# joaospinto/sip_optimal_control

Hardware: AMD Instinct MI355X
Metric: Riccati sweeps/sec (backward+forward) (higher is better)
Workload: dtype f64

## Files before the change

sip_optimal_control_amd/csrc/chain_qw16.hpp:

```cpp
#pragma once
#include <hip/hip_runtime.h>
#include <type_traits>

#include "dpp_blocks_gen.hpp"

namespace sipamd {

template <int I, int E, class F>
__device__ __forceinline__ void sfor(F &&f) {
  if constexpr (I < E) {
    f(std::integral_constant<int, I>{});
    sfor<I + 1, E>(f);
  }
}
template <int I, int E, class F>
__device__ __forceinline__ void sfor_down(F &&f) {
  if constexpr (I > E) {
    f(std::integral_constant<int, I>{});
    sfor_down<I - 1, E>(f);
  }
}

template <int K>
__device__ __forceinline__ double bcast(double x) {
  double und;
  asm volatile("" : "=v"(und));
  return __builtin_amdgcn_update_dpp(und, x, 0x150 + K, 0xf, 0xf, false);
}

__device__ __forceinline__ double rsqrt_nr(double d) {
  const double y = __builtin_amdgcn_rsq(d);
  const double s = d * y;
  const double e = __builtin_fma(-s, y, 1.0);
  const double t = __builtin_fma(0.375, e, 0.5);
  return __builtin_fma(y * e, t, y);
}

__device__ __forceinline__ double rcp_nr(double d) {
  const double y = __builtin_amdgcn_rcp(d);
  const double e = __builtin_fma(-d, y, 1.0);
  const double t = __builtin_fma(e, e, e);
  return __builtin_fma(y, t, y);
}

template <int S>
__device__ __forceinline__ bool chol_ldl_dpp(double (&A)[S], double (&dinv)[S],
                                             const int c) {
#ifdef SIP_QW16_CHOL_SELECT
  unsigned long long failmask = 0;
  sfor<0, S>([&](auto kk) {
    constexpr int k = decltype(kk)::value;
    const double d = bcast<k>(A[k]);
    failmask |= __ballot(d <= 0.0);
    const double y2 = rcp_nr(d);
    dinv[k] = y2;
    const double upd = (c > k && c < S) ? A[k] * y2 : 0.0;
    rank1<S - k - 1, k, true, false>(A + k + 1, A + k + 1, upd);
  });
  return ((failmask >> (__lane_id() & 63)) & 1ull) != 0;
#else
  double dmin = __builtin_inf();
  sfor<0, S>([&](auto kk) {
    constexpr int k = decltype(kk)::value;
    const double d = bcast<k>(A[k]);
    asm("v_min_f64 %0, %1, %2" : "=v"(dmin) : "v"(dmin), "v"(d));
    const double own = A[k] * ((c > k && c < S) ? 1.0 : 0.0);
    const double y2 = rcp_nr(d);
    dinv[k] = y2;
    const double upd = own * y2;
    rank1<S - k - 1, k, true, false>(A + k + 1, A + k + 1, upd);
  });
  return dmin <= 0.0;
#endif
}

template <int S>
__device__ __forceinline__ void ldl_solve_dpp(const double (&Lt)[S],
                                              const double (&dinv)[S],
                                              double (&X)[S]) {
  sfor<0, S>([&](auto jj) {
    constexpr int j = decltype(jj)::value;
    X[j] *= dinv[j];
    rank1<S - j - 1, j, true, (j == 0)>(X + j + 1, Lt + j + 1, X[j]);
  });
  double acc[S];
  sfor<0, S>([&](auto jj) { acc[decltype(jj)::value] = 0.0; });
  sfor_down<S - 1, -1>([&](auto jj) {
    constexpr int j = decltype(jj)::value;
    X[j] = __builtin_fma(-dinv[j], acc[j], X[j]);
    spread<j, false, false>(acc, Lt[j], X[j]);
  });
}

template <int N, int M, bool SYM = false>
struct ChainLayout {
  static constexpr int QLEN = SYM ? N * (N + 1) / 2 : N * N;
  static constexpr int RLEN = SYM ? M * (M + 1) / 2 : M * M;
  static constexpr int NODE = QLEN + N;
  static constexpr int EDGE = N * N + 2 * N * M + RLEN;
  static constexpr int VNODE = 2 * N;
  static constexpr int VEDGE = M;
  static constexpr int GAIN = M * N + M;
  static constexpr int WSN = N * N + 2 * N;
};

template <int N, bool EXPORT = false>
__device__ __forceinline__ bool node_factor(const double (&V)[N], const double dl,
                                            const int c, const double (&E)[N],
                                            const double (&tv)[N], double (&W)[N],
                                            double (&X)[N], double *Lt = nullptr) {
  const double sdi = rsqrt_nr(dl);
  const double sd = dl * sdi;
  double S[N], A[N], rinv[N];
  sfor<0, N>([&](auto ii) { S[decltype(ii)::value] = 0.0; });
  spread<N, false, true>(S, sd, sd);
  sfor<0, N>([&](auto ii) {
    constexpr int r = decltype(ii)::value;
    A[r] = __builtin_fma(S[r], V[r], E[r]);
  });
  const bool fail = chol_ldl_dpp<N>(A, rinv, c);
  if constexpr (EXPORT)
    sfor<0, N>([&](auto ii) { Lt[decltype(ii)::value] = A[decltype(ii)::value]; });
  sfor<0, N>([&](auto ii) { X[decltype(ii)::value] = E[decltype(ii)::value]; });
  spreadv<N, false>(X, sdi, tv);
  ldl_solve_dpp<N>(A, rinv, X);
  sfor<0, N>([&](auto ii) { S[decltype(ii)::value] = 0.0; });
  spread<N, false, true>(S, sdi, sdi);
  sfor<0, N>([&](auto ii) {
    constexpr int r = decltype(ii)::value;
    W[r] = (E[r] - X[r]) * S[r];
  });
  return fail;
}

#ifndef SIP_LQR_NT_SOL
#define SIP_LQR_NT_SOL 0
#endif
#ifndef SIP_LQR_NT_IN
#define SIP_LQR_NT_IN 2
#endif
#ifndef SIP_LQR_NT_FAB
#define SIP_LQR_NT_FAB SIP_LQR_NT_IN
#endif
#ifndef SIP_LQR_NT_FSP
#define SIP_LQR_NT_FSP 0
#endif
typedef __attribute__((address_space(3))) char lds_char;
typedef const __attribute__((address_space(3))) double lds_cdouble;

#ifdef SIP_LQR_STAMPS
#define SIP_STAMP(var)                                                         \
  do {                                                                         \
    __builtin_amdgcn_sched_barrier(0);                                         \
    asm volatile("s_memtime %0\n\ts_waitcnt lgkmcnt(0)" : "=s"(var)::"memory"); \
    __builtin_amdgcn_sched_barrier(0);                                         \
  } while (0)
#define SIP_STAMP_ARG , unsigned long long *__restrict__ stamps
#define SIP_SEG(k)                                                             \
  do {                                                                         \
    unsigned long long now_;                                                   \
    SIP_STAMP(now_);                                                           \
    seg[k] += now_ - seg_last;                                                 \
    seg_last = now_;                                                           \
  } while (0)
#else
#define SIP_SEG(k)                                                             \
  do {                                                                         \
  } while (0)
#define SIP_STAMP(var)                                                         \
  do {                                                                         \
  } while (0)
#define SIP_STAMP_ARG
#endif

template <int PIECES>
struct StageDma {
  static constexpr int INSTR = (4 * PIECES + 63) / 64;
  static constexpr int BYTES = INSTR * 1024;
  static constexpr int ROW_BYTES = PIECES * 16;
#ifdef SIP_QW16_DMA_PLAIN
  static constexpr int GROUP = 1;
#else
  static constexpr int GROUP = 4;
#endif
  static constexpr unsigned BIAS = (GROUP - 1) * 1024u;
  unsigned off[INSTR > 0 ? INSTR : 1];
  __device__ __forceinline__ void init(const int lane,
                                       const unsigned problem_stride_bytes,
                                       const unsigned max_rel) {
    sfor<0, INSTR>([&](auto jj) {
      constexpr int j = decltype(jj)::value;
      const unsigned q = (unsigned)(j * 64 + lane) < 4u * PIECES ? (unsigned)(j * 64 + lane) : 4u * PIECES - 1u;
      unsigned rr = q / PIECES;
      const unsigned within = q - rr * PIECES;
      rr = rr < max_rel ? rr : max_rel;
      off[j] = rr * problem_stride_bytes + within * 16u + BIAS - (unsigned)(j % GROUP) * 1024u;
    });
  }
  template <int AUX = 0>
  __device__ __forceinline__ void issue(const char *base, lds_char *dst,
                                        const int lane) const {
    const char *lowered = base - BIAS;
    sfor<0, INSTR>([&](auto jj) {
      constexpr int j = decltype(jj)::value;
      __builtin_amdgcn_global_load_lds((const __attribute__((address_space(1))) void *)(lowered + off[j]),
                                       (__attribute__((address_space(3))) void *)(dst + (j - j % GROUP) * 1024), 16,
                                       (j % GROUP) * 1024, AUX);
    });
  }
};

template <int DWORDS>
struct StageDmaDwords {
  static constexpr int INSTR = (4 * DWORDS + 63) / 64;
  static constexpr int BYTES = (INSTR * 256 + 1023) / 1024 * 1024;
  static constexpr int ROW_BYTES = DWORDS * 4;
  unsigned off[INSTR > 0 ? INSTR : 1];
  __device__ __forceinline__ void init(const int lane, const unsigned problem_stride_bytes, const unsigned max_rel) {
    sfor<0, INSTR>([&](auto jj) {
      constexpr int j = decltype(jj)::value;
      const unsigned q = (unsigned)(j * 64 + lane) < 4u * DWORDS ? (unsigned)(j * 64 + lane) : 4u * DWORDS - 1u;
      unsigned rr = q / DWORDS;
      const unsigned within = q - rr * DWORDS;
      rr = rr < max_rel ? rr : max_rel;
      off[j] = rr * problem_stride_bytes + within * 4u;
    });
  }
  template <int AUX = 0>
  __device__ __forceinline__ void issue(const char *base, lds_char *dst, const int lane) const {
    sfor<0, INSTR>([&](auto jj) {
      constexpr int j = decltype(jj)::value;
      __builtin_amdgcn_global_load_lds((const __attribute__((address_space(1))) void *)(base + off[j]),
                                       (__attribute__((address_space(3))) void *)(dst + j * 256), 4, 0, AUX);
    });
  }
};

template <int PIECES>
struct StageDmaRows {
  static constexpr int IP = (PIECES + 63) / 64;
  static constexpr int INSTR = 4 * IP;
  static constexpr int ROW_BYTES = IP * 1024;
  static constexpr int BYTES = 4 * ROW_BYTES;
  static constexpr bool RAGGED = PIECES % 64 != 0;
  unsigned vo_main, vo_tail;
  unsigned long long row[4];
  __device__ __forceinline__ void init(const int lane,
                                       const unsigned problem_stride_bytes,
                                       const unsigned max_rel) {
    vo_main = (unsigned)lane * 16u;
    const unsigned last = (unsigned)(PIECES - 1 - 64 * (IP - 1));
    vo_tail = ((unsigned)lane < last ? (unsigned)lane : last) * 16u;
    sfor<0, 4>([&](auto rq) {
      constexpr unsigned r = decltype(rq)::value;
      row[r] = (unsigned long long)(r < max_rel ? r : max_rel) * problem_stride_bytes;
    });
  }
  template <int AUX = 0>
  __device__ __forceinline__ void issue(const char *base, lds_char *dst,
                                        const int lane) const {
    sfor<0, 4>([&](auto rq) {
      constexpr int r = decltype(rq)::value;
      const char *region = base + row[r];
      sfor<0, IP>([&](auto jq) {
        constexpr int jj = decltype(jq)::value;
        constexpr int g = jj / 4;
        const unsigned vo = (RAGGED && jj == IP - 1) ? vo_tail : vo_main;
        __builtin_amdgcn_global_load_lds(
            (const __attribute__((address_space(1))) void *)(region + g * 4096 + vo),
            (__attribute__((address_space(3))) void *)(dst + r * ROW_BYTES + g * 4096), 16, (jj % 4) * 1024, AUX);
      });
    });
  }
};

template <int N, int M, bool WPACK, bool SPLIT = false, bool SYM = false>
struct StagedCfg {
  using L = ChainLayout<N, M, SYM>;
  static_assert(!SYM || (L::QLEN % 2 == 0 && L::RLEN % 2 == 0 && N % 2 == 0 && M % 2 == 0),
                "the symmetric-packed kernels are instantiated where every block stays a whole number of 16-byte pieces");
  static constexpr int AB = N * N + N * M;
  static constexpr int STG = L::NODE + L::EDGE - (SPLIT ? AB : 0);
  static constexpr int WSN =
      WPACK ? ((N * (N + 1) / 2 + 2 * N + 1) / 2) * 2 : L::WSN;
  using BV = StageDma<(L::VNODE + L::VEDGE + 1) / 2>;
  using BMflat = StageDma<(STG + 1) / 2>;
  using BMrows = StageDmaRows<(STG + 1) / 2>;
  struct NoStream {
    static constexpr int INSTR = 0, BYTES = 0, ROW_BYTES = 0;
  };
  static_assert(!SPLIT || AB % 2 == 0, "the split kernels are instantiated for even N (A | B in whole 16-byte pieces)");
  using BA = std::conditional_t<SPLIT, StageDmaRows<AB / 2>, NoStream>;
  static constexpr int SCR_BYTES_ = ((4 * 2 * N + N) * 8 + 1023) / 1024 * 1024;
  static constexpr int waves_per_cu(int bm_bytes) {
    const int per_wave = 2 * (bm_bytes + BA::BYTES + BV::BYTES) + SCR_BYTES_;
    const int w = 163840 / per_wave;
    return w > 4 ? 4 : w;
  }
#ifdef SIP_QW16_DMA_FLAT
  using BM = BMflat;
#else
  using BM = std::conditional_t<SPLIT || waves_per_cu(BMrows::BYTES) >= waves_per_cu(BMflat::BYTES), BMrows, BMflat>;
#endif
  static constexpr int B_BYTES = BM::BYTES + BA::BYTES + BV::BYTES;
  using FA = StageDma<(N * N + N * M + 1) / 2>;
  using FG = std::conditional_t<L::GAIN % 2 == 0, StageDma<L::GAIN / 2>, StageDmaDwords<2 * L::GAIN>>;
  using FW = StageDma<WSN / 2>;
  using FC = std::conditional_t<N % 2 == 0, StageDma<N / 2>, StageDmaDwords<2 * N>>;
  static constexpr int F_BYTES = FA::BYTES + FG::BYTES + FW::BYTES + FC::BYTES;
  static constexpr int F_GLDS = FA::INSTR + FG::INSTR + FW::INSTR + FC::INSTR;
  static constexpr int B_NBUF = 2;
  static constexpr int lds_main(int fbufs) {
    return B_NBUF * B_BYTES > fbufs * F_BYTES ? B_NBUF * B_BYTES : fbufs * F_BYTES;
  }
  static constexpr int waves_with(int fbufs) {
    const int w = 163840 / (lds_main(fbufs) + SCR_BYTES_);
    return w > 4 ? 4 : w;
  }
#ifdef SIP_LQR_FNBUF
  static constexpr int F_NBUF = SIP_LQR_FNBUF;
#else
  static constexpr int F_NBUF = (waves_with(2) > waves_with(3) || lds_main(3) + SCR_BYTES_ > 65536) ? 2 : 3;
#endif
  static constexpr int LDS_MAIN = lds_main(F_NBUF);
  static constexpr int SCR_BYTES = ((4 * 2 * N + N) * 8 + 1023) / 1024 * 1024;
  static constexpr int LDS_BYTES = LDS_MAIN + SCR_BYTES;
  static constexpr bool OK = N <= 16;
  static constexpr bool WIDE = N % 2 == 0;
};

template <int N, int M, bool STAGED, bool WPACK, bool SPLIT = false, bool SYM = false>
__global__ __launch_bounds__(64) void chain_factor_solve_qw16(
    const double *__restrict__ mats, const double *__restrict__ vecs,
    double *__restrict__ sol, double *__restrict__ gains,
    double *__restrict__ wsp, int *__restrict__ status, const long batch,
    const int T, const int mode, double *__restrict__ gfac,
    const double *__restrict__ ab, const long ab_pstride, const long ab_sstride SIP_STAMP_ARG) {
  constexpr bool VDIST = N == 16;
  static_assert(N >= 1 && N <= 16, "one problem per 16-lane row");
  static_assert(M >= 1 && M <= 16, "");
  using L = ChainLayout<N, M, SYM>;
  using C = StagedCfg<N, M, WPACK, SPLIT, SYM>;
  static_assert(!SPLIT || (STAGED && WPACK), "the split kernel is the staged one");
  static_assert(!SYM || (STAGED && !VDIST), "the symmetric-packed layout is served by the staged kernels");
  unsigned long long ts_begin = 0, ts_term = 0, ts_bwd = 0, ts_root = 0,
                     ts_end = 0, ts_a = 0, ts_b = 0, acc_bwait = 0,
                     acc_fwait = 0;
  (void)ts_begin, (void)ts_term, (void)ts_bwd, (void)ts_root, (void)ts_end,
      (void)ts_a, (void)ts_b, (void)acc_bwait, (void)acc_fwait;
  unsigned long long seg[12] = {0, 0, 0, 0, 0, 0, 0, 0, 0, 0, 0, 0}, seg_last = 0;
  (void)seg, (void)seg_last;
  SIP_STAMP(ts_begin);
  static_assert(!STAGED || C::LDS_BYTES <= 65536, "the LDS images of this shape exceed a workgroup's 64 KiB");
  constexpr int STG = C::STG;
  constexpr int OFF_M = L::NODE + (SPLIT ? 0 : N * N + N * M), OFF_R = OFF_M + N * M;
  constexpr int VSTG = L::VNODE + L::VEDGE;
  constexpr int WSN = C::WSN;
  constexpr int WG = WPACK ? N * (N + 1) / 2 : N * N;

  extern __shared__ double lds_raw[];
  lds_char *const lds = (lds_char *)lds_raw;

  const int lane = threadIdx.x & 63;
  const int c = lane & 15;
  const int rr = lane >> 4;
  const long p0 = (long)blockIdx.x * 4;
  long p = p0 + rr;
  const bool valid = p < batch;
  if (!valid)
    p = batch - 1;
  const bool isM = c < N;
  const bool isV = c == N;
  const int cm = isM ? c : N - 1;
  const int cu = c < M ? c : M - 1;

  const long mats_len = (long)(T + 1) * L::NODE + (long)T * (STG - L::NODE);
  const long vecs_len = (long)(T + 1) * L::VNODE + (long)T * L::VEDGE;
  const long gains_len = (long)T * L::GAIN;
  const long ws_len = (long)(T + 1) * WSN;
  const double *pm = mats + p * mats_len;
  const double *pv = vecs + p * vecs_len;
  double *ps = sol + p * vecs_len;
  double *pg = gains + p * gains_len;
  double *pw = wsp + p * ws_len;
  const unsigned max_rel =
      (unsigned)((batch - 1 - p0) < 3 ? (batch - 1 - p0) : 3);

  double E[N];
  sfor<0, N>([&](auto ii) {
    constexpr int r = decltype(ii)::value;
    E[r] = (c == r) ? 1.0 : 0.0;
  });

  auto spill_row_offsets = [&](int(&woff)[N]) {
    sfor<0, N>([&](auto kk) {
      constexpr int k = decltype(kk)::value;
      if constexpr (WPACK) {
        const int lo = k < cm ? k : cm, hi = k < cm ? cm : k;
        woff[k] = lo * N - (lo * (lo - 1)) / 2 + (hi - lo);
      } else {
        woff[k] = cm * N + k;
      }
    });
  };

  int stat = 0;
  double W[N], V[N], t[N], vch[N];
  double vd = 0.0, td = 0.0, qd = 0.0;
  auto sum4 = [](const double (&a)[4]) { return (a[0] + a[1]) + (a[2] + a[3]); };

  const __amdgpu_buffer_rsrc_t ws_rsrc = __builtin_amdgcn_make_buffer_rsrc(
      (void *)(wsp + p0 * ws_len), 0, (int)((max_rel + 1) * ws_len * 8), 0x00020000);
  const int wstore_base = (valid && isM)
                              ? (int)(rr * ws_len * 8) + (c * N - (c * (c - 1)) / 2 - c) * 8
                              : 0x7ffff000;

  typedef __attribute__((address_space(3))) double lds_double;
  lds_char *const scr = lds + C::LDS_MAIN;
  lds_double *const my_t = (lds_double *)(scr + rr * (2 * N * 8));
  lds_double *const my_v = my_t + N;
  lds_cdouble *const zeros = (lds_cdouble *)(scr + 4 * (2 * N * 8));
  if constexpr (STAGED) {
    if (lane < N)
      ((lds_double *)zeros)[lane] = 0.0;
  }

  auto load_vq = [&](auto nm, auto nv, double(&Vq)[N]) {
    if constexpr (SYM) {
      const int base_c = cm * N - (cm * (cm - 1)) / 2 - cm;
      sfor<0, N>([&](auto ii) {
        constexpr int r = decltype(ii)::value;
        constexpr int base_r = r * N - (r * (r - 1)) / 2 - r;
        const int off = r >= cm ? base_c + r : base_r + cm;
        auto src = isV ? nv + r : nm + off;
        Vq[r] = *src;
      });
    } else {
    auto src = isV ? nv : nm + cm * N;
    sfor<0, N>([&](auto ii) {
      constexpr int r = decltype(ii)::value;
      Vq[r] = src[r];
    });
    }
    if constexpr (VDIST)
      qd = nv[cm];
  };

  struct NodeTail {
    double dl, cv[N], dv[N];
    double cd;
  };
  auto load_tail = [&](auto nm, auto nv, NodeTail &nt) {
    const double d = nm[L::QLEN + cm];
    nt.dl = isM ? d : 1.0;
    nt.cd = VDIST ? nv[N + cm] : 0.0;
    if constexpr (std::is_same_v<decltype(nm), lds_cdouble *>) {
      auto csrc = isV ? nv + N : zeros, dsrc = isV ? nm + L::QLEN : zeros;
      sfor<0, N>([&](auto ii) {
        constexpr int r = decltype(ii)::value;
        nt.cv[r] = csrc[r];
        nt.dv[r] = dsrc[r];
      });
    } else {
      sfor<0, N>([&](auto ii) {
        constexpr int r = decltype(ii)::value;
        nt.cv[r] = isV ? nv[N + r] : 0.0;
        nt.dv[r] = isV ? nm[L::QLEN + r] : 0.0;
      });
    }
  };
  auto finish_node = [&](const int i, const NodeTail &nt) {
    const double dl = nt.dl;
    const unsigned long long bad = __ballot(isM && dl <= 0.0);
    const bool bad_row = ((bad >> (lane & 48)) & 0xffffull) != 0;
    if (stat == 0 && bad_row)
      stat = 1;
    double tv[N], X[N];
    sfor<0, N>([&](auto ii) {
      constexpr int r = decltype(ii)::value;
      tv[r] = nt.cv[r] - nt.dv[r] * V[r];
    });
    if constexpr (STAGED && C::WIDE) {
      if (isV) {
        typedef double d2 __attribute__((ext_vector_type(2)));
        typedef __attribute__((address_space(3))) d2 lds_d2;
        lds_d2 *const t2 = (lds_d2 *)my_t, *const v2 = (lds_d2 *)my_v;
        sfor<0, N / 2>([&](auto kk) {
          constexpr int k = decltype(kk)::value;
          t2[k] = d2{tv[2 * k], tv[2 * k + 1]};
          v2[k] = d2{V[2 * k], V[2 * k + 1]};
        });
      }
    } else if constexpr (STAGED) {
      if (isV) {
        sfor<0, N>([&](auto ii) {
          constexpr int r = decltype(ii)::value;
          my_t[r] = tv[r];
          my_v[r] = V[r];
        });
      }
    } else {
      sfor<0, N>([&](auto ii) {
        constexpr int r = decltype(ii)::value;
        t[r] = tv[r];
        vch[r] = V[r];
      });
    }
    if constexpr (VDIST)
      td = nt.cd - dl * vd;
    SIP_SEG(7);
    const bool ffail = node_factor<N>(V, dl, c, E, tv, W, X);
    SIP_SEG(8);
    if (stat == 0 && ffail)
      stat = 2;
    if constexpr (VDIST) {
      const double phi = rsqrt_nr(dl) * td;
      double acc[4] = {0.0, 0.0, 0.0, 0.0};
      dotv<N, true>(acc, phi, X);
      if (valid)
        pw[(long)i * WSN + WG + N + c] = sum4(acc);
    }
    if (valid && isV) {
      double *hn = pw + (long)i * WSN + WG + N;
      sfor<0, N>([&](auto ii) { hn[decltype(ii)::value] = X[decltype(ii)::value]; });
    }
    if constexpr (WPACK) {
      sfor<0, N>([&](auto ii) {
        constexpr int r = decltype(ii)::value;
        const int vo = (r >= c) ? wstore_base : 0x7ffff000;
        typedef unsigned int u32x2 __attribute__((ext_vector_type(2)));
        __builtin_amdgcn_raw_buffer_store_b64(__builtin_bit_cast(u32x2, X[r]), ws_rsrc, vo + r * 8,
                                              i * (WSN * 8), 0);
      });
    } else if (valid && isM) {
      double *wn = pw + (long)i * WSN + c * N;
      sfor<0, N>(
          [&](auto ii) { wn[decltype(ii)::value] = X[decltype(ii)::value]; });
    }
  };

  auto backward_edge = [&](const int i, auto nm, auto ea, auto nv, NodeTail &nt) {

    double F[N], Aaug[N], Bcol[N];
    double Hc[M], G[M], rinvG[M], H[M], K[M];
    {
      auto msrc = isV ? nv + L::VNODE : nm + (OFF_M + cm);
      sfor<0, M>([&](auto jj) {
        constexpr int j = decltype(jj)::value;
        if constexpr (SYM) {
          const int lo = j < cu ? j : cu, hi = j < cu ? cu : j;
          G[j] = nm[OFF_R + lo * M - (lo * (lo - 1)) / 2 + (hi - lo)];
        } else
        G[j] = nm[OFF_R + cu * M + j];
        H[j] = isV ? msrc[j] : msrc[j * N];
      });
    }
    if constexpr (STAGED && C::WIDE) {
      typedef double d2 __attribute__((ext_vector_type(2)));
      typedef const __attribute__((address_space(3))) d2 lds_cd2;
      lds_cd2 *a_src = (lds_cd2 *)(isV ? (lds_cdouble *)my_t : ea + cm * N);
      lds_cd2 *f_src = (lds_cd2 *)(isV ? (lds_cdouble *)my_v : zeros);
      lds_cd2 *b_src = (lds_cd2 *)(ea + N * N + cu * N);
      sfor<0, N / 2>([&](auto kk) {
        constexpr int k = decltype(kk)::value;
        const d2 a2 = a_src[k], f2 = f_src[k], b2 = b_src[k];
        Aaug[2 * k] = a2[0], Aaug[2 * k + 1] = a2[1];
        F[2 * k] = f2[0], F[2 * k + 1] = f2[1];
        Bcol[2 * k] = b2[0], Bcol[2 * k + 1] = b2[1];
      });
    } else if constexpr (STAGED) {
      lds_cdouble *a_src = isV ? (lds_cdouble *)my_t : ea + cm * N;
      lds_cdouble *f_src = isV ? (lds_cdouble *)my_v : zeros;
      lds_cdouble *b_src = ea + N * N + cu * N;
      sfor<0, N>([&](auto kk) {
        constexpr int k = decltype(kk)::value;
        Aaug[k] = a_src[k], F[k] = f_src[k], Bcol[k] = b_src[k];
      });
    } else {
      sfor<0, N>([&](auto kk) {
        constexpr int k = decltype(kk)::value;
        Aaug[k] = isV ? t[k] : ea[cm * N + k];
        F[k] = isV ? vch[k] : 0.0;
        Bcol[k] = ea[N * N + cu * N + k];
      });
    }
    rank1x<N, N, true>(F, W, Aaug);
    if (valid && isV) {
      double *gn = pw + (long)(i + 1) * WSN + WG;
      sfor<0, N>(
          [&](auto ii) { gn[decltype(ii)::value] = F[decltype(ii)::value]; });
    }
    double gd = 0.0, hd = 0.0, hf[M], kf[M];
    if constexpr (VDIST) {
      double acc[4] = {0.0, 0.0, 0.0, 0.0};
      dotv<N, true>(acc, td, W);
      gd = vd + sum4(acc);
      if (valid)
        pw[(long)(i + 1) * WSN + WG + c] = gd;
    }
    SIP_SEG(2);
    asm volatile("" ::: "memory");
    double Vn[N];
    load_vq(nm, nv, Vn);

    sfor<0, M>([&](auto jj) { Hc[decltype(jj)::value] = 0.0; });
    spreadx<M, N, false>(Hc, Bcol, W);
    rank1x<M, N, true>(G, Hc, Bcol);
    SIP_SEG(3);
    const bool gfail = chol_ldl_dpp<M>(G, rinvG, c);
    if (mode == 1 && valid) {
      double *gf = gfac + (p * (long)T + i) * (M * M + M);
      if (c < M)
        sfor<0, M>([&](auto jj) { gf[c * M + decltype(jj)::value] = G[decltype(jj)::value]; });
      if (c == 0)
        sfor<0, M>([&](auto jj) { gf[M * M + decltype(jj)::value] = rinvG[decltype(jj)::value]; });
    }
    SIP_SEG(4);
    if (stat == 0 && gfail)
      stat = 3;

    spreadx<M, N, false>(H, Bcol, F);
    if constexpr (VDIST) {
      double acc[4] = {0.0, 0.0, 0.0, 0.0};
      dotv<N, true>(acc, gd, Bcol);
      hd = nv[L::VNODE + cu] + sum4(acc);
    }
    sfor<0, M>(
        [&](auto jj) { K[decltype(jj)::value] = H[decltype(jj)::value]; });
    ldl_solve_dpp<M>(G, rinvG, K);
    sfor<0, M>(
        [&](auto jj) { K[decltype(jj)::value] = -K[decltype(jj)::value]; });
    if (valid && c <= N) {
      double *gi = pg + (long)i * L::GAIN + c * M;
      sfor<0, M>(
          [&](auto jj) { gi[decltype(jj)::value] = K[decltype(jj)::value]; });
    }
    if constexpr (VDIST) {
      double Lf[M][M];
      sfor<0, M>([&](auto jj) {
        constexpr int j = decltype(jj)::value;
        hf[j] = bcast<j>(hd);
        sfor<0, j>([&](auto iv) {
          constexpr int i2 = decltype(iv)::value;
          Lf[j][i2] = bcast<i2>(G[j]);
        });
      });
      sfor<0, M>([&](auto jj) {
        constexpr int j = decltype(jj)::value;
        double w = hf[j];
        sfor<0, j>([&](auto iv) { w = __builtin_fma(-Lf[j][decltype(iv)::value], kf[decltype(iv)::value], w); });
        kf[j] = w * rinvG[j];
      });
      sfor_down<M - 1, -1>([&](auto jj) {
        constexpr int j = decltype(jj)::value;
        double a = 0.0;
        sfor<j + 1, M>([&](auto iv) { a = __builtin_fma(Lf[decltype(iv)::value][j], kf[decltype(iv)::value], a); });
        kf[j] = __builtin_fma(-rinvG[j], a, kf[j]);
      });
      sfor<0, M>([&](auto jj) { kf[decltype(jj)::value] = -kf[decltype(jj)::value]; });
      if (valid && c == 0) {
        double *gk = pg + (long)i * L::GAIN + N * M;
        sfor<0, M>([&](auto jj) { gk[decltype(jj)::value] = kf[decltype(jj)::value]; });
      }
    }

    SIP_SEG(5);
    spreadx<N, N, false>(Vn, Aaug, F);
    asm volatile("" ::: "memory");
    load_tail(nm, nv, nt);
    asm volatile("" ::: "memory");
    spreadx<N, M, true>(Vn, K, H);
    sfor<0, N>(
        [&](auto ii) { V[decltype(ii)::value] = Vn[decltype(ii)::value]; });
    if constexpr (VDIST) {
      double acc[4] = {0.0, 0.0, 0.0, 0.0};
      dotv<N, true>(acc, gd, Aaug);
      double kh = 0.0;
      sfor<0, M>([&](auto jj) { kh = __builtin_fma(K[decltype(jj)::value], hf[decltype(jj)::value], kh); });
      vd = qd + sum4(acc) + kh;
    }
    SIP_SEG(6);
    asm volatile("" ::: "memory");
  };

  if (mode != 2) {
  typename C::BM dma_bm;
  typename C::BA dma_ba;
  typename C::BV dma_bv;
  auto issue_backward = [&](const int i, lds_char *buf) {
    dma_bm.template issue<SIP_LQR_NT_IN>((const char *)(mats + p0 * mats_len + (long)i * STG), buf, lane);
    if constexpr (SPLIT)
      dma_ba.template issue<SIP_LQR_NT_IN>((const char *)(ab + p0 * ab_pstride + (long)i * ab_sstride),
                                           buf + C::BM::BYTES, lane);
    dma_bv.template issue<SIP_LQR_NT_IN>((const char *)(vecs + p0 * vecs_len + (long)i * VSTG),
                                         buf + C::BM::BYTES + C::BA::BYTES, lane);
  };
  if constexpr (STAGED) {
    dma_bm.init(lane, (unsigned)(mats_len * 8), max_rel);
    if constexpr (SPLIT)
      dma_ba.init(lane, (unsigned)(ab_pstride * 8), max_rel);
    dma_bv.init(lane, (unsigned)(vecs_len * 8), max_rel);
    if (T > 0)
      issue_backward(T - 1, lds + ((T - 1) & 1) * C::B_BYTES);
  }
  {
    NodeTail nt;
    load_vq(pm + (long)T * STG, pv + (long)T * VSTG, V);
    if constexpr (VDIST)
      vd = qd;
    load_tail(pm + (long)T * STG, pv + (long)T * VSTG, nt);
    finish_node(T, nt);
  }
  SIP_STAMP(ts_term);

  auto stage_step = [&](const int i, auto par) {
    SIP_STAMP(ts_a);
#ifdef SIP_LQR_STAMPS
    seg_last = ts_a;
    if (stamps != nullptr && lane == 0 && i < 64)
      stamps[(long)gridDim.x * 24 + (long)blockIdx.x * 128 + i] = ts_a;
#endif
    if constexpr (STAGED) {
      constexpr int PAR = decltype(par)::value;
      lds_char *buf = lds + PAR * C::B_BYTES;
      if constexpr (WPACK)
        asm volatile("s_waitcnt vmcnt(%0)" ::"n"(N) : "memory");
      else
        asm volatile("s_waitcnt vmcnt(0)" ::: "memory");
      SIP_STAMP(ts_b);
      acc_bwait += ts_b - ts_a;
      SIP_SEG(0);
      if (i > 0) {
        issue_backward(i - 1, lds + (PAR ^ 1) * C::B_BYTES);
        asm volatile("" ::: "memory");
      }
      lds_cdouble *nm = (lds_cdouble *)(buf + rr * C::BM::ROW_BYTES);
      lds_cdouble *ea = SPLIT ? (lds_cdouble *)(buf + C::BM::BYTES + rr * C::BA::ROW_BYTES) : nm + L::NODE;
      lds_cdouble *nv = (lds_cdouble *)(buf + C::BM::BYTES + C::BA::BYTES + rr * C::BV::ROW_BYTES);
      SIP_SEG(1);
      NodeTail nt;
      backward_edge(i, nm, ea, nv, nt);
      finish_node(i, nt);
    } else {
      const double *nm = pm + (long)i * STG;
      const double *nv = pv + (long)i * VSTG;
      SIP_SEG(1);
      NodeTail nt;
      backward_edge(i, nm, nm + L::NODE, nv, nt);
      finish_node(i, nt);
    }
    SIP_SEG(9);
  };
#ifdef SIP_QW16_NO_PARITY_UNROLL
  constexpr bool kParityUnroll = false;
#else
  constexpr bool kParityUnroll = STAGED;
#endif
  if constexpr (kParityUnroll) {
    for (int i = (T - 1) | 1; i >= 1; i -= 2) {
      if (i <= T - 1)
        stage_step(i, std::integral_constant<int, 1>{});
      stage_step(i - 1, std::integral_constant<int, 0>{});
    }
  } else if constexpr (STAGED) {
    for (int i = T - 1; i >= 0; --i) {
      if (i & 1)
        stage_step(i, std::integral_constant<int, 1>{});
      else
        stage_step(i, std::integral_constant<int, 0>{});
    }
  } else {
    for (int i = T - 1; i >= 0; --i)
      stage_step(i, std::integral_constant<int, 0>{});
  }

  SIP_STAMP(ts_bwd);
  if constexpr (VDIST) {
    double acc[4] = {0.0, 0.0, 0.0, 0.0};
    dotv<N, true>(acc, td, W);
    if (valid)
      pw[WG + c] = vd + sum4(acc);
  } else {
    double F[N], tt[N];
    sfor<0, N>([&](auto ii) {
      constexpr int r = decltype(ii)::value;
      if constexpr (STAGED) {
        tt[r] = isV ? my_t[r] : 0.0;
        F[r] = isV ? my_v[r] : 0.0;
      } else {
        tt[r] = t[r];
        F[r] = vch[r];
      }
    });
    rank1x<N, N, true>(F, W, tt);
    if (valid && isV) {
      double *gn = pw + WG;
      sfor<0, N>([&](auto ii) { gn[decltype(ii)::value] = F[decltype(ii)::value]; });
    }
  }
  if (valid && c == 0)
    status[p] = stat;
  } else if constexpr (!SPLIT) {
    int woff[N];
    spill_row_offsets(woff);
    auto node_step = [&](const int i, const double v_) {
      const double dl = pm[(long)i * STG + L::QLEN + cm];
      const double t_ = pv[(long)i * VSTG + N + cm] - dl * v_;
      const double sdi = rsqrt_nr(dl);
      const double phi = sdi * t_;
      const double *slot = pw + (long)i * WSN;
      double Srow[N];
      sfor<0, N>([&](auto kk) { Srow[decltype(kk)::value] = slot[woff[decltype(kk)::value]]; });
      double acc[4] = {0.0, 0.0, 0.0, 0.0};
      dotv<N, true>(acc, phi, Srow);
      const double sphi = sum4(acc);
      if (valid && isM)
        pw[(long)i * WSN + WG + N + c] = sphi;
      return sdi * (phi - sphi);
    };
    double v_ = pv[(long)T * VSTG + cm];
    double wt = node_step(T, v_);
    for (int i = T - 1; i >= 0; --i) {
      const double *em = pm + (long)i * STG + L::NODE;
      const double *gi = pg + (long)i * L::GAIN;
      const double *gf = gfac + (p * (long)T + i) * (M * M + M);
      const double gd = v_ + wt;
      if (valid && isM)
        pw[(long)(i + 1) * WSN + WG + c] = gd;
      double Bcol[N], Acol[N], Kc[M], hf[M], kf[M], Lf[M][M], rinv[M];
      sfor<0, N>([&](auto kk) {
        constexpr int k = decltype(kk)::value;
        Bcol[k] = em[N * N + cu * N + k];
        Acol[k] = em[cm * N + k];
      });
      sfor<0, M>([&](auto jj) {
        constexpr int j = decltype(jj)::value;
        Kc[j] = gi[cm * M + j];
        rinv[j] = gf[M * M + j];
        sfor<0, j>([&](auto iv) { Lf[j][decltype(iv)::value] = gf[decltype(iv)::value * M + j]; });
      });
      double acc[4] = {0.0, 0.0, 0.0, 0.0};
      dotv<N, true>(acc, gd, Bcol);
      const double hd = pv[(long)i * VSTG + L::VNODE + cu] + sum4(acc);
      sfor<0, M>([&](auto jj) { hf[decltype(jj)::value] = bcast<decltype(jj)::value>(hd); });
      sfor<0, M>([&](auto jj) {
        constexpr int j = decltype(jj)::value;
        double w = hf[j];
        sfor<0, j>([&](auto iv) { w = __builtin_fma(-Lf[j][decltype(iv)::value], kf[decltype(iv)::value], w); });
        kf[j] = w * rinv[j];
      });
      sfor_down<M - 1, -1>([&](auto jj) {
        constexpr int j = decltype(jj)::value;
        double a = 0.0;
        sfor<j + 1, M>([&](auto iv) { a = __builtin_fma(Lf[decltype(iv)::value][j], kf[decltype(iv)::value], a); });
        kf[j] = __builtin_fma(-rinv[j], a, kf[j]);
      });
      if (valid && c == 0) {
        double *gk = pg + (long)i * L::GAIN + N * M;
        sfor<0, M>([&](auto jj) { gk[decltype(jj)::value] = -kf[decltype(jj)::value]; });
      }
      double acc2[4] = {0.0, 0.0, 0.0, 0.0};
      dotv<N, true>(acc2, gd, Acol);
      double kh = 0.0;
      sfor<0, M>([&](auto jj) { kh = __builtin_fma(Kc[decltype(jj)::value], hf[decltype(jj)::value], kh); });
      v_ = pv[(long)i * VSTG + cm] + sum4(acc2) + kh;
      wt = node_step(i, v_);
    }
    if (valid && isM)
      pw[WG + c] = v_ + wt;
  }

  if (mode == 1)
    return;
  __syncthreads();
  SIP_STAMP(ts_root);


  typename C::FA dma_fa;
  typename C::FG dma_fg;
  typename C::FW dma_fw;
  typename C::FC dma_fd;
  if constexpr (STAGED) {
    dma_fa.init(lane, (unsigned)((SPLIT ? ab_pstride : mats_len) * 8), max_rel);
    dma_fg.init(lane, (unsigned)(gains_len * 8), max_rel);
    dma_fw.init(lane, (unsigned)(ws_len * 8), max_rel);
    dma_fd.init(lane, (unsigned)(mats_len * 8), max_rel);
  }
  auto issue_forward = [&](const int i, lds_char *buf) {
    dma_fa.template issue<SIP_LQR_NT_FAB>(
        (const char *)(SPLIT ? ab + p0 * ab_pstride + (long)i * ab_sstride : mats + p0 * mats_len + (long)i * STG + L::NODE),
        buf, lane);
    dma_fg.template issue<SIP_LQR_NT_FSP>((const char *)(gains + p0 * gains_len + (long)i * L::GAIN),
                 buf + C::FA::BYTES, lane);
    dma_fw.template issue<SIP_LQR_NT_FSP>((const char *)(wsp + p0 * ws_len + (long)(i + 1) * WSN),
                 buf + C::FA::BYTES + C::FG::BYTES, lane);
    dma_fd.template issue<SIP_LQR_NT_FAB>(
        (const char *)(mats + p0 * mats_len + (long)(i + 1) * STG + L::QLEN),
        buf + C::FA::BYTES + C::FG::BYTES + C::FW::BYTES, lane);
  };
  if constexpr (STAGED) {
    if (T > 0)
      issue_forward(0, lds);
    if (C::F_NBUF == 3 && T > 1)
      issue_forward(1, lds + C::F_BYTES);
  }

  double x, y;
  {
    const double gg = pw[WG + cm];
    const double hh = pw[WG + N + cm];
    const double dd = pm[L::QLEN + cm];
    y = gg;
    x = (dd * rsqrt_nr(dd)) * hh;
    if (valid && isM) {
      ps[c] = x;
      ps[N + c] = y;
    }
  }
  int woff[N];
  spill_row_offsets(woff);
  int fbuf = 0;
  for (int i = 0; i < T; ++i) {
    double KT[N], Arow[N], Brow[M], Wc[N];
    double kk0, gg, hh, dd;
    auto read_stage = [&](auto em, auto gi, auto wn, auto dp) {
      sfor<0, N>([&](auto kk) {
        constexpr int k = decltype(kk)::value;
        KT[k] = gi[k * M + cu];
        Arow[k] = em[k * N + cm];
        Wc[k] = wn[woff[k]];
      });
      sfor<0, M>([&](auto jj) {
        constexpr int j = decltype(jj)::value;
        Brow[j] = em[N * N + j * N + cm];
      });
      kk0 = gi[N * M + cu];
      gg = wn[WG + cm];
      hh = wn[WG + N + cm];
      dd = dp[cm];
    };
    SIP_STAMP(ts_a);
#ifdef SIP_LQR_STAMPS
    if (stamps != nullptr && lane == 0 && i < 64)
      stamps[(long)gridDim.x * 24 + (long)blockIdx.x * 128 + 64 + i] = ts_a;
#endif
    if constexpr (STAGED) {
      lds_char *buf = lds + (fbuf * C::F_BYTES);
      static_assert(C::F_GLDS < 64, "vmcnt is 6 bits");
      if (C::F_NBUF == 3 && i + 1 < T)
        asm volatile("s_waitcnt vmcnt(%0)" ::"n"(C::F_GLDS) : "memory");
      else
        asm volatile("s_waitcnt vmcnt(0)" ::: "memory");
      SIP_STAMP(ts_b);
      acc_fwait += ts_b - ts_a;
      lds_char *b1 = buf + C::FA::BYTES, *b2 = b1 + C::FG::BYTES,
               *b3 = b2 + C::FW::BYTES;
      read_stage((lds_cdouble *)(buf + rr * C::FA::ROW_BYTES),
                 (lds_cdouble *)(b1 + rr * C::FG::ROW_BYTES),
                 (lds_cdouble *)(b2 + rr * (WSN * 8)),
                 (lds_cdouble *)(b3 + rr * C::FC::ROW_BYTES));
      asm volatile("s_waitcnt lgkmcnt(0)" ::: "memory");
      if (C::F_NBUF == 2 && i + 1 < T)
        issue_forward(i + 1, lds + (fbuf ^ 1) * C::F_BYTES);
    } else {
      read_stage(pm + (long)i * STG + L::NODE, pg + (long)i * L::GAIN,
                 pw + (long)(i + 1) * WSN, pm + (long)(i + 1) * STG + L::QLEN);
    }

    const double sdi = rsqrt_nr(dd), sdv = dd * sdi;
    double acc[4];
    acc[0] = kk0, acc[1] = 0.0, acc[2] = 0.0, acc[3] = 0.0;
    dotv<N, true>(acc, x, KT);
    const double u = (acc[0] + acc[1]) + (acc[2] + acc[3]);
    acc[0] = 0.0, acc[1] = 0.0, acc[2] = 0.0, acc[3] = 0.0;
    dotv<N, true>(acc, x, Arow);
    dotv<M, true>(acc, u, Brow);
    const double z = (acc[0] + acc[1]) + (acc[2] + acc[3]);
    const double zeta = z * sdi;
    acc[0] = 0.0, acc[1] = 0.0, acc[2] = 0.0, acc[3] = 0.0;
    dotv<N, true>(acc, zeta, Wc);
    const double sz = (acc[0] + acc[1]) + (acc[2] + acc[3]);
    x = sdv * (sz + hh);
    y = __builtin_fma(sdi, zeta - sz, gg);
    if (valid) {
      double *si = ps + (long)i * VSTG;
#if SIP_LQR_NT_SOL
      if (c < M)
        __builtin_nontemporal_store(u, si + 2 * N + c);
      if (isM) {
        __builtin_nontemporal_store(x, si + VSTG + c);
        __builtin_nontemporal_store(y, si + VSTG + N + c);
      }
#else
      if (c < M)
        si[2 * N + c] = u;
      if (isM) {
        si[VSTG + c] = x;
        si[VSTG + N + c] = y;
      }
#endif
    }
    if constexpr (STAGED) {
      asm volatile("" ::: "memory");
      const int nbuf = fbuf >= 1 ? fbuf - 1 : C::F_NBUF - 1;
      if (C::F_NBUF == 3 && i + 2 < T)
        issue_forward(i + 2, lds + nbuf * C::F_BYTES);
      fbuf = fbuf + 1 == C::F_NBUF ? 0 : fbuf + 1;
    }
  }
#ifdef SIP_LQR_STAMPS
  SIP_STAMP(ts_end);
  if (stamps != nullptr && lane == 0) {
    unsigned long long *o = stamps + (long)blockIdx.x * 24;
    o[0] = ts_begin, o[1] = ts_term, o[2] = ts_bwd, o[3] = ts_root;
    o[4] = ts_end, o[5] = acc_bwait, o[6] = acc_fwait;
    o[7] = __builtin_amdgcn_s_memrealtime();
    for (int k = 0; k < 12; ++k)
      o[8 + k] = seg[k];
  }
#endif
}

}
```

Before: 13.40 million.

## Defer RHS solve to forward rollout and shrink per-stage workspace

The backward sweep no longer solves the node right-hand side or stores the g/h vectors. It stores only the factor rows plus the vd/V vector, which cuts the workspace from N*N+2N to N*N+N per stage. The forward rollout rebuilds zeta from z, the stored v and a newly staged c vector, and adds one extra DMA stream for c. Solution stores move to buffer stores, with vmcnt accounting adjusted so they stay in flight. This trades backward-pass work and storage for a slightly larger forward stage, and the changed waitcnt arithmetic risks subtle ordering bugs.

```diff
diff --git a/sip_optimal_control_amd/csrc/chain_qw16.hpp b/sip_optimal_control_amd/csrc/chain_qw16.hpp
--- a/sip_optimal_control_amd/csrc/chain_qw16.hpp
+++ b/sip_optimal_control_amd/csrc/chain_qw16.hpp
@@ -43,7 +43,7 @@
   return __builtin_fma(y, t, y);
 }
 
-template <int S>
+template <int S, bool WAIT0 = false>
 __device__ __forceinline__ bool chol_ldl_dpp(double (&A)[S], double (&dinv)[S],
                                              const int c) {
 #ifdef SIP_QW16_CHOL_SELECT
@@ -55,7 +55,7 @@
     const double y2 = rcp_nr(d);
     dinv[k] = y2;
     const double upd = (c > k && c < S) ? A[k] * y2 : 0.0;
-    rank1<S - k - 1, k, true, false>(A + k + 1, A + k + 1, upd);
+    rank1<S - k - 1, k, true, (WAIT0 && k == 0)>(A + k + 1, A + k + 1, upd);
   });
   return ((failmask >> (__lane_id() & 63)) & 1ull) != 0;
 #else
@@ -68,7 +68,7 @@
     const double y2 = rcp_nr(d);
     dinv[k] = y2;
     const double upd = own * y2;
-    rank1<S - k - 1, k, true, false>(A + k + 1, A + k + 1, upd);
+    rank1<S - k - 1, k, true, (WAIT0 && k == 0)>(A + k + 1, A + k + 1, upd);
   });
   return dmin <= 0.0;
 #endif
@@ -101,10 +101,10 @@
   static constexpr int VNODE = 2 * N;
   static constexpr int VEDGE = M;
   static constexpr int GAIN = M * N + M;
-  static constexpr int WSN = N * N + 2 * N;
+  static constexpr int WSN = N * N + N;
 };
 
-template <int N, bool EXPORT = false>
+template <int N, bool EXPORT = false, bool RHS = true>
 __device__ __forceinline__ bool node_factor(const double (&V)[N], const double dl,
                                             const int c, const double (&E)[N],
                                             const double (&tv)[N], double (&W)[N],
@@ -118,11 +118,12 @@
     constexpr int r = decltype(ii)::value;
     A[r] = __builtin_fma(S[r], V[r], E[r]);
   });
-  const bool fail = chol_ldl_dpp<N>(A, rinv, c);
+  const bool fail = chol_ldl_dpp<N, !RHS>(A, rinv, c);
   if constexpr (EXPORT)
     sfor<0, N>([&](auto ii) { Lt[decltype(ii)::value] = A[decltype(ii)::value]; });
   sfor<0, N>([&](auto ii) { X[decltype(ii)::value] = E[decltype(ii)::value]; });
-  spreadv<N, false>(X, sdi, tv);
+  if constexpr (RHS)
+    spreadv<N, false>(X, sdi, tv);
   ldl_solve_dpp<N>(A, rinv, X);
   sfor<0, N>([&](auto ii) { S[decltype(ii)::value] = 0.0; });
   spread<N, false, true>(S, sdi, sdi);
@@ -282,7 +283,7 @@
   static constexpr int AB = N * N + N * M;
   static constexpr int STG = L::NODE + L::EDGE - (SPLIT ? AB : 0);
   static constexpr int WSN =
-      WPACK ? ((N * (N + 1) / 2 + 2 * N + 1) / 2) * 2 : L::WSN;
+      WPACK ? ((N * (N + 1) / 2 + N + 1) / 2) * 2 : L::WSN;
   using BV = StageDma<(L::VNODE + L::VEDGE + 1) / 2>;
   using BMflat = StageDma<(STG + 1) / 2>;
   using BMrows = StageDmaRows<(STG + 1) / 2>;
@@ -307,8 +308,10 @@
   using FG = std::conditional_t<L::GAIN % 2 == 0, StageDma<L::GAIN / 2>, StageDmaDwords<2 * L::GAIN>>;
   using FW = StageDma<WSN / 2>;
   using FC = std::conditional_t<N % 2 == 0, StageDma<N / 2>, StageDmaDwords<2 * N>>;
-  static constexpr int F_BYTES = FA::BYTES + FG::BYTES + FW::BYTES + FC::BYTES;
-  static constexpr int F_GLDS = FA::INSTR + FG::INSTR + FW::INSTR + FC::INSTR;
+  using FCV = std::conditional_t<N % 2 == 0 && M % 2 == 0, StageDma<N / 2>, StageDmaDwords<2 * N>>;
+  static constexpr int F_BYTES = FA::BYTES + FG::BYTES + FW::BYTES + FC::BYTES + FCV::BYTES;
+  static constexpr int F_GLDS = FA::INSTR + FG::INSTR + FW::INSTR + FC::INSTR + FCV::INSTR;
+  static constexpr int F_STORES = 3;
   static constexpr int B_NBUF = 2;
   static constexpr int lds_main(int fbufs) {
     return B_NBUF * B_BYTES > fbufs * F_BYTES ? B_NBUF * B_BYTES : fbufs * F_BYTES;
@@ -380,7 +383,6 @@
   const long ws_len = (long)(T + 1) * WSN;
   const double *pm = mats + p * mats_len;
   const double *pv = vecs + p * vecs_len;
-  double *ps = sol + p * vecs_len;
   double *pg = gains + p * gains_len;
   double *pw = wsp + p * ws_len;
   const unsigned max_rel =
@@ -411,9 +413,14 @@
 
   const __amdgpu_buffer_rsrc_t ws_rsrc = __builtin_amdgcn_make_buffer_rsrc(
       (void *)(wsp + p0 * ws_len), 0, (int)((max_rel + 1) * ws_len * 8), 0x00020000);
-  const int wstore_base = (valid && isM)
-                              ? (int)(rr * ws_len * 8) + (c * N - (c * (c - 1)) / 2 - c) * 8
+  const int wstore_base = (valid && c <= N)
+                              ? (int)(rr * ws_len * 8) + (isV ? WG : c * N - (c * (c - 1)) / 2 - c) * 8
                               : 0x7ffff000;
+  const int wstore_first = isV ? 0 : c;
+  const __amdgpu_buffer_rsrc_t sol_rsrc = __builtin_amdgcn_make_buffer_rsrc(
+      (void *)(sol + p0 * vecs_len), 0, (int)((max_rel + 1) * vecs_len * 8), 0x00020000);
+  const int sol_u = (valid && c < M) ? (int)(rr * vecs_len * 8) + (2 * N + c) * 8 : 0x7ffff000;
+  const int sol_x = (valid && isM) ? (int)(rr * vecs_len * 8) + c * 8 : 0x7ffff000;
 
   typedef __attribute__((address_space(3))) double lds_double;
   lds_char *const scr = lds + C::LDS_MAIN;
@@ -509,33 +516,28 @@
     if constexpr (VDIST)
       td = nt.cd - dl * vd;
     SIP_SEG(7);
-    const bool ffail = node_factor<N>(V, dl, c, E, tv, W, X);
+    const bool ffail = node_factor<N, false, false>(V, dl, c, E, E, W, X);
     SIP_SEG(8);
     if (stat == 0 && ffail)
       stat = 2;
     if constexpr (VDIST) {
-      const double phi = rsqrt_nr(dl) * td;
-      double acc[4] = {0.0, 0.0, 0.0, 0.0};
-      dotv<N, true>(acc, phi, X);
       if (valid)
-        pw[(long)i * WSN + WG + N + c] = sum4(acc);
-    }
-    if (valid && isV) {
-      double *hn = pw + (long)i * WSN + WG + N;
-      sfor<0, N>([&](auto ii) { hn[decltype(ii)::value] = X[decltype(ii)::value]; });
+        pw[(long)i * WSN + WG + c] = vd;
     }
     if constexpr (WPACK) {
       sfor<0, N>([&](auto ii) {
         constexpr int r = decltype(ii)::value;
-        const int vo = (r >= c) ? wstore_base : 0x7ffff000;
+        const int vo = (r >= wstore_first) ? wstore_base : 0x7ffff000;
         typedef unsigned int u32x2 __attribute__((ext_vector_type(2)));
-        __builtin_amdgcn_raw_buffer_store_b64(__builtin_bit_cast(u32x2, X[r]), ws_rsrc, vo + r * 8,
+        __builtin_amdgcn_raw_buffer_store_b64(__builtin_bit_cast(u32x2, isV ? V[r] : X[r]), ws_rsrc, vo + r * 8,
                                               i * (WSN * 8), 0);
       });
-    } else if (valid && isM) {
-      double *wn = pw + (long)i * WSN + c * N;
-      sfor<0, N>(
-          [&](auto ii) { wn[decltype(ii)::value] = X[decltype(ii)::value]; });
+    } else if (valid && c <= N) {
+      double *wn = pw + (long)i * WSN + (isV ? WG : c * N);
+      sfor<0, N>([&](auto ii) {
+        constexpr int r = decltype(ii)::value;
+        wn[r] = isV ? V[r] : X[r];
+      });
     }
   };
 
@@ -585,18 +587,11 @@
       });
     }
     rank1x<N, N, true>(F, W, Aaug);
-    if (valid && isV) {
-      double *gn = pw + (long)(i + 1) * WSN + WG;
-      sfor<0, N>(
-          [&](auto ii) { gn[decltype(ii)::value] = F[decltype(ii)::value]; });
-    }
     double gd = 0.0, hd = 0.0, hf[M], kf[M];
     if constexpr (VDIST) {
       double acc[4] = {0.0, 0.0, 0.0, 0.0};
       dotv<N, true>(acc, td, W);
       gd = vd + sum4(acc);
-      if (valid)
-        pw[(long)(i + 1) * WSN + WG + c] = gd;
     }
     SIP_SEG(2);
     asm volatile("" ::: "memory");
@@ -775,29 +770,6 @@
   }
 
   SIP_STAMP(ts_bwd);
-  if constexpr (VDIST) {
-    double acc[4] = {0.0, 0.0, 0.0, 0.0};
-    dotv<N, true>(acc, td, W);
-    if (valid)
-      pw[WG + c] = vd + sum4(acc);
-  } else {
-    double F[N], tt[N];
-    sfor<0, N>([&](auto ii) {
-      constexpr int r = decltype(ii)::value;
-      if constexpr (STAGED) {
-        tt[r] = isV ? my_t[r] : 0.0;
-        F[r] = isV ? my_v[r] : 0.0;
-      } else {
-        tt[r] = t[r];
-        F[r] = vch[r];
-      }
-    });
-    rank1x<N, N, true>(F, W, tt);
-    if (valid && isV) {
-      double *gn = pw + WG;
-      sfor<0, N>([&](auto ii) { gn[decltype(ii)::value] = F[decltype(ii)::value]; });
-    }
-  }
   if (valid && c == 0)
     status[p] = stat;
   } else if constexpr (!SPLIT) {
@@ -815,7 +787,7 @@
       dotv<N, true>(acc, phi, Srow);
       const double sphi = sum4(acc);
       if (valid && isM)
-        pw[(long)i * WSN + WG + N + c] = sphi;
+        pw[(long)i * WSN + WG + c] = v_;
       return sdi * (phi - sphi);
     };
     double v_ = pv[(long)T * VSTG + cm];
@@ -825,8 +797,6 @@
       const double *gi = pg + (long)i * L::GAIN;
       const double *gf = gfac + (p * (long)T + i) * (M * M + M);
       const double gd = v_ + wt;
-      if (valid && isM)
-        pw[(long)(i + 1) * WSN + WG + c] = gd;
       double Bcol[N], Acol[N], Kc[M], hf[M], kf[M], Lf[M][M], rinv[M];
       sfor<0, N>([&](auto kk) {
         constexpr int k = decltype(kk)::value;
@@ -866,8 +836,6 @@
       v_ = pv[(long)i * VSTG + cm] + sum4(acc2) + kh;
       wt = node_step(i, v_);
     }
-    if (valid && isM)
-      pw[WG + c] = v_ + wt;
   }
 
   if (mode == 1)
@@ -880,11 +848,13 @@
   typename C::FG dma_fg;
   typename C::FW dma_fw;
   typename C::FC dma_fd;
+  typename C::FCV dma_fc;
   if constexpr (STAGED) {
     dma_fa.init(lane, (unsigned)((SPLIT ? ab_pstride : mats_len) * 8), max_rel);
     dma_fg.init(lane, (unsigned)(gains_len * 8), max_rel);
     dma_fw.init(lane, (unsigned)(ws_len * 8), max_rel);
     dma_fd.init(lane, (unsigned)(mats_len * 8), max_rel);
+    dma_fc.init(lane, (unsigned)(vecs_len * 8), max_rel);
   }
   auto issue_forward = [&](const int i, lds_char *buf) {
     dma_fa.template issue<SIP_LQR_NT_FAB>(
@@ -897,6 +867,9 @@
     dma_fd.template issue<SIP_LQR_NT_FAB>(
         (const char *)(mats + p0 * mats_len + (long)(i + 1) * STG + L::QLEN),
         buf + C::FA::BYTES + C::FG::BYTES + C::FW::BYTES, lane);
+    dma_fc.template issue<SIP_LQR_NT_FAB>(
+        (const char *)(vecs + p0 * vecs_len + (long)(i + 1) * VSTG + N),
+        buf + C::FA::BYTES + C::FG::BYTES + C::FW::BYTES + C::FC::BYTES, lane);
   };
   if constexpr (STAGED) {
     if (T > 0)
@@ -905,25 +878,32 @@
       issue_forward(1, lds + C::F_BYTES);
   }
 
-  double x, y;
-  {
-    const double gg = pw[WG + cm];
-    const double hh = pw[WG + N + cm];
-    const double dd = pm[L::QLEN + cm];
-    y = gg;
-    x = (dd * rsqrt_nr(dd)) * hh;
-    if (valid && isM) {
-      ps[c] = x;
-      ps[N + c] = y;
-    }
-  }
   int woff[N];
   spill_row_offsets(woff);
+  typedef unsigned int u32x2 __attribute__((ext_vector_type(2)));
+  constexpr int SOL_AUX = SIP_LQR_NT_SOL ? 2 : 0;
+  double x, y;
+  auto rollout_node = [&](const double z, const double vv, const double cc, const double dd, const double(&Srow)[N]) {
+    const double sdi = rsqrt_nr(dd), sdv = dd * sdi;
+    const double zeta = (z + __builtin_fma(-dd, vv, cc)) * sdi;
+    double acc[4] = {0.0, 0.0, 0.0, 0.0};
+    dotv<N, true>(acc, zeta, Srow);
+    const double sz = sum4(acc);
+    x = sdv * sz;
+    y = __builtin_fma(sdi, zeta - sz, vv);
+  };
+  {
+    double Srow[N];
+    sfor<0, N>([&](auto kk) { Srow[decltype(kk)::value] = pw[woff[decltype(kk)::value]]; });
+    rollout_node(0.0, pw[WG + cm], pv[N + cm], pm[L::QLEN + cm], Srow);
+    __builtin_amdgcn_raw_buffer_store_b64(__builtin_bit_cast(u32x2, x), sol_rsrc, sol_x, 0, SOL_AUX);
+    __builtin_amdgcn_raw_buffer_store_b64(__builtin_bit_cast(u32x2, y), sol_rsrc, sol_x + N * 8, 0, SOL_AUX);
+  }
   int fbuf = 0;
   for (int i = 0; i < T; ++i) {
     double KT[N], Arow[N], Brow[M], Wc[N];
-    double kk0, gg, hh, dd;
-    auto read_stage = [&](auto em, auto gi, auto wn, auto dp) {
+    double kk0, vv, cc, dd;
+    auto read_stage = [&](auto em, auto gi, auto wn, auto dp, auto cp) {
       sfor<0, N>([&](auto kk) {
         constexpr int k = decltype(kk)::value;
         KT[k] = gi[k * M + cu];
@@ -935,9 +915,9 @@
         Brow[j] = em[N * N + j * N + cm];
       });
       kk0 = gi[N * M + cu];
-      gg = wn[WG + cm];
-      hh = wn[WG + N + cm];
+      vv = wn[WG + cm];
       dd = dp[cm];
+      cc = cp[cm];
     };
     SIP_STAMP(ts_a);
 #ifdef SIP_LQR_STAMPS
@@ -946,28 +926,33 @@
 #endif
     if constexpr (STAGED) {
       lds_char *buf = lds + (fbuf * C::F_BYTES);
-      static_assert(C::F_GLDS < 64, "vmcnt is 6 bits");
-      if (C::F_NBUF == 3 && i + 1 < T)
+      static_assert(C::F_GLDS + C::F_STORES < 64, "vmcnt is 6 bits");
+      if (C::F_NBUF == 3 && i > 0) {
+        if (i + 1 < T)
+          asm volatile("s_waitcnt vmcnt(%0)" ::"n"(C::F_GLDS + C::F_STORES) : "memory");
+        else
+          asm volatile("s_waitcnt vmcnt(%0)" ::"n"(C::F_STORES) : "memory");
+      } else if (C::F_NBUF == 3 && i + 1 < T)
         asm volatile("s_waitcnt vmcnt(%0)" ::"n"(C::F_GLDS) : "memory");
       else
         asm volatile("s_waitcnt vmcnt(0)" ::: "memory");
       SIP_STAMP(ts_b);
       acc_fwait += ts_b - ts_a;
       lds_char *b1 = buf + C::FA::BYTES, *b2 = b1 + C::FG::BYTES,
-               *b3 = b2 + C::FW::BYTES;
+               *b3 = b2 + C::FW::BYTES, *b4 = b3 + C::FC::BYTES;
       read_stage((lds_cdouble *)(buf + rr * C::FA::ROW_BYTES),
                  (lds_cdouble *)(b1 + rr * C::FG::ROW_BYTES),
                  (lds_cdouble *)(b2 + rr * (WSN * 8)),
-                 (lds_cdouble *)(b3 + rr * C::FC::ROW_BYTES));
+                 (lds_cdouble *)(b3 + rr * C::FC::ROW_BYTES),
+                 (lds_cdouble *)(b4 + rr * C::FCV::ROW_BYTES));
       asm volatile("s_waitcnt lgkmcnt(0)" ::: "memory");
       if (C::F_NBUF == 2 && i + 1 < T)
         issue_forward(i + 1, lds + (fbuf ^ 1) * C::F_BYTES);
     } else {
       read_stage(pm + (long)i * STG + L::NODE, pg + (long)i * L::GAIN,
-                 pw + (long)(i + 1) * WSN, pm + (long)(i + 1) * STG + L::QLEN);
-    }
-
-    const double sdi = rsqrt_nr(dd), sdv = dd * sdi;
+                 pw + (long)(i + 1) * WSN, pm + (long)(i + 1) * STG + L::QLEN, pv + (long)(i + 1) * VSTG + N);
+    }
+
     double acc[4];
     acc[0] = kk0, acc[1] = 0.0, acc[2] = 0.0, acc[3] = 0.0;
     dotv<N, true>(acc, x, KT);
@@ -976,30 +961,11 @@
     dotv<N, true>(acc, x, Arow);
     dotv<M, true>(acc, u, Brow);
     const double z = (acc[0] + acc[1]) + (acc[2] + acc[3]);
-    const double zeta = z * sdi;
-    acc[0] = 0.0, acc[1] = 0.0, acc[2] = 0.0, acc[3] = 0.0;
-    dotv<N, true>(acc, zeta, Wc);
-    const double sz = (acc[0] + acc[1]) + (acc[2] + acc[3]);
-    x = sdv * (sz + hh);
-    y = __builtin_fma(sdi, zeta - sz, gg);
-    if (valid) {
-      double *si = ps + (long)i * VSTG;
-#if SIP_LQR_NT_SOL
-      if (c < M)
-        __builtin_nontemporal_store(u, si + 2 * N + c);
-      if (isM) {
-        __builtin_nontemporal_store(x, si + VSTG + c);
-        __builtin_nontemporal_store(y, si + VSTG + N + c);
-      }
-#else
-      if (c < M)
-        si[2 * N + c] = u;
-      if (isM) {
-        si[VSTG + c] = x;
-        si[VSTG + N + c] = y;
-      }
-#endif
-    }
+    rollout_node(z, vv, cc, dd, Wc);
+    const int so = i * (VSTG * 8);
+    __builtin_amdgcn_raw_buffer_store_b64(__builtin_bit_cast(u32x2, u), sol_rsrc, sol_u, so, SOL_AUX);
+    __builtin_amdgcn_raw_buffer_store_b64(__builtin_bit_cast(u32x2, x), sol_rsrc, sol_x + VSTG * 8, so, SOL_AUX);
+    __builtin_amdgcn_raw_buffer_store_b64(__builtin_bit_cast(u32x2, y), sol_rsrc, sol_x + (VSTG + N) * 8, so, SOL_AUX);
     if constexpr (STAGED) {
       asm volatile("" ::: "memory");
       const int nbuf = fbuf >= 1 ? fbuf - 1 : C::F_NBUF - 1;
```

Result: no change. 13.68 million (median of 6 runs) (+2.1%).
